# DeepRank/Deeprank-GNN

Measured on AMD Instinct MI355X. Metric: interface-graphs/sec (fwd+bwd) GINet batch=64 per GPU, higher is better.
Workload: dtype f32; 1 GPU; GINet train step (topology + body fwd + FC head/MSE + bwd + grad all-reduce + Adam) on SYN graphs: 200 nodes, ~1000 directed edges, 32 node feats, 50->16 clusters (BASELINE.json configs[1]); graphs_per_gpu=64, global_batch=64, parallelism=dp1, mode=native, step_layout=auto

## Files before the change

deeprank-gnn_amd/csrc/drgnn_capi.hip:

```cpp
#define DRGNN_KERNELS_MAIN
#include "drgnn_kernels.h"

#include <vector>
#include <algorithm>
#include <memory>
#include <string.h>
#include <stdlib.h>
#ifdef DRGNN_EMU
#define DRGNN_LDS_LIMIT (160 * 1024)
#else
#define DRGNN_LDS_LIMIT (160 * 1024)
#define HIP_TRY(expr)                                   \
    do {                                                \
        hipError_t e_ = (expr);                         \
        if (e_ != hipSuccess) return (int)e_;           \
    } while (0)
#endif



extern "C" {

int drgnn_abi_version(void) { return DRGNN_ABI_VERSION; }

// ... 1477 lines not shown
        if (int rc = head_width_check(d)) return rc;
    }
    if (int rc = net_check(d.net)) return rc;
    if (!d.g_conv1 || !d.g_conv2 || slabs_check(d.net, c.slabs.slabs_per_graph)) return DRGNN_E_ARG;
    if (c.cohort) return 0;
    if (c.options) { if (int rc = optim_check(c.optim)) return rc; }
    if (!c.slabs.conv_partials || !c.slabs.head_partials || !c.flat.grad) return DRGNN_E_ARG;
    if (d.compact && (!c.slabs.readout || !c.step2)) return DRGNN_E_ARG;
    if (c.apply_adam && (!c.flat.param || !c.flat.exp_avg || !c.flat.exp_avg_sq || (!d.compact && !c.step))) return DRGNN_E_ARG;
    return 0;
}
static void reduce_fill(ReduceArgs& r, const drgnn_net_desc* net, const float* partials, int64_t rows, const drgnn_conv_grads* g1,
                        const drgnn_conv_grads* g2) {
    r = ReduceArgs{};
    r.partials = partials; r.n_graphs = (int)rows; r.n_branch = net->n_branch;
    r.n_feat = net->n_feat; r.n_partial = (int)net_partial_floats(net->n_feat); r.kind = net->kind;
    for (int b = 0; b < DRGNN_MAX_BRANCH; ++b) { r.lay1[b] = net->conv1[b]; r.lay2[b] = net->conv2[b]; }
    for (int b = 0; b < net->n_branch; ++b) { r.g1[b] = g1[b]; r.g2[b] = g2[b]; }
}
static int update_sums_fill(UpdateArgs& u, const UpdateDst& d, const UpdateSlabs& s, int n_tail) {
    reduce_fill(u.r, d.net, s.conv_partials, slabs_split(d.net, s.slabs_per_graph) ? 2 * s.n_graphs : s.n_graphs, d.g_conv1, d.g_conv2);
    u.h.partials = s.head_partials; u.h.n_wg = (int)s.head_slabs;
    u.h.P = (int)(d.compact ? head_compact_floats(d.R, d.H, d.O) : head_partial_floats(d.R, d.H, d.O));
    u.readout = s.readout; u.hR = d.R; u.hH = d.H;
    u.blocks_per_branch = (u.r.n_partial + 63) / 64;
    u.conv_blocks = d.net->n_branch * u.blocks_per_branch;
    return (d.compact ? d.H * d.R : 0) + u.h.P - n_tail;
}

static int update_run(const UpdateCall& c) {
    if (int rc = update_check(c)) return rc;
    UpdateArgs u = {};
    const int head_items = update_sums_fill(u, c.dst, c.slabs, 1);
    const int n_blocks = u.conv_blocks + (head_items + 63) / 64;
    if (!c.cohort) { u.h.grad = c.flat.grad + c.flat.head_offset; u.ad.step = c.dst.compact ? c.step2 + 1 : c.step; }
    u.h.loss = c.loss; u.loss2 = (c.loss || c.cohort) ? c.loss2 : nullptr; u.step2 = c.dst.compact ? c.step2 : nullptr;
    u.ad.param = c.flat.param; u.ad.grad = c.flat.grad; u.ad.exp_avg = c.flat.exp_avg; u.ad.exp_avg_sq = c.flat.exp_avg_sq;
    u.ad.n = c.flat.n_param;
    const drgnn_optim* opt = c.apply_adam ? c.optim : nullptr;
    const bool opt_flat = opt && (opt->clip || optim_coupled(opt));
    if (c.optim) optim_adam_args(u.ad, c.optim);
    else adam_set_hyper(u.ad, c.lr, c.beta1, c.beta2, c.eps, 0.0);
    u.apply_adam = (c.apply_adam && !opt_flat) ? 1 : 0;
#ifdef DRGNN_EMU
    if (c.cohort) return DRGNN_E_CAPACITY;
    if (opt) u.apply_adam = 0;
    const ReduceArgs& r = u.r;
    for (int64_t i = 0; i < (int64_t)r.n_branch * r.n_partial; ++i) {
        const int br = (int)(i / r.n_partial), p = (int)(i % r.n_partial);
        if (!reduce_live(r, p)) continue;
        float* d = reduce_dst(r, br, p);
        if (d) update_store(u, d, reduce_sum(r, br, p, 0, 1));
    }
    for (int i = 0; i < head_items; ++i) update_head_store(u, i, update_head_sum(u, i, 0, 1));
    if (u.step2) u.step2[0] = u.step2[1];
    if (opt) return adam_opt_impl(u.ad, c.flat.grad, opt, 0, c.stream);
#else
    const dim3 grid((unsigned)n_blocks, c.cohort ? (unsigned)c.K : 1u), threads(DRGNN_UPDATE_THREADS);
    hipStream_t stream = (hipStream_t)c.stream;
    if (opt) {
        const bool words = opt->clip && !optim_coupled(opt);
        if (words && n_blocks > opt->norm_cap) return DRGNN_E_CAPACITY;
        hipLaunchKernelGGL(k_update_opt, grid, threads, 0, stream, u, *opt, words ? opt->norm_words : (double*)nullptr);
        HIP_TRY(hipGetLastError());
        return opt_flat ? adam_opt_impl(u.ad, c.flat.grad, opt, words ? n_blocks : 0, c.stream) : 0;
    }
    if (c.optims) {
        if (c.any_clip && n_blocks > drgnn_optim_norm_words(c.flat.n_param)) return DRGNN_E_CAPACITY;
// ... 44 lines not shown
    return 0;
}

extern "C" {

int drgnn_net_reduce_grads(const drgnn_net_desc* net, const float* partials, int64_t n_nodes, int64_t n_graphs,
                           drgnn_conv_grads* g_conv1, drgnn_conv_grads* g_conv2, float* grad_x, void* stream_) {
    if (int rc = net_check(net)) return rc;
    if (!partials || !g_conv1 || !g_conv2) return DRGNN_E_ARG;
    ReduceArgs r;
    reduce_fill(r, net, partials, n_graphs, g_conv1, g_conv2);
    r.grad_x = grad_x; r.n_nodes = n_nodes;
    int64_t items = (int64_t)net->n_branch * r.n_partial;
    if (grad_x && net->n_branch > 1 && n_nodes * net->n_feat > items) items = n_nodes * net->n_feat;
#ifdef DRGNN_EMU
    for (int64_t i = 0; i < (int64_t)net->n_branch * r.n_partial; ++i) {
        const int br = (int)(i / r.n_partial), p = (int)(i % r.n_partial);
        if (reduce_live(r, p)) reduce_write(r, br, p, reduce_sum(r, br, p, 0, 1));
    }
    for (int64_t i = 0; grad_x && i < n_nodes * net->n_feat; ++i) reduce_grad_x(r, i);
    (void)stream_; (void)items;
#else
    const int reduce_blocks = net->n_branch * ((r.n_partial + 63) / 64);
    hipLaunchKernelGGL(k_reduce, dim3((unsigned)reduce_blocks), dim3(256), 0, (hipStream_t)stream_, r, items);
    HIP_TRY(hipGetLastError());
#endif
    return 0;
}

int drgnn_train_update(const drgnn_net_desc* net, const float* conv_partials, int64_t n_graphs, drgnn_conv_grads* g_conv1,
                       drgnn_conv_grads* g_conv2, const float* head_partials, int64_t head_slabs, int32_t R, int32_t H, int32_t O,
                       int64_t head_offset, float* flat_param, float* flat_grad, float* exp_avg, float* exp_avg_sq, int64_t n_param,
                       const int32_t* step, float* loss, double lr, double beta1, double beta2, double eps, int32_t apply_adam,
                       void* stream_) {
    UpdateCall c = update_call({net, g_conv1, g_conv2, R, H, O, false}, {conv_partials, n_graphs, head_partials, head_slabs, nullptr, 0},
                               {flat_param, flat_grad, exp_avg, exp_avg_sq, n_param, head_offset}, loss, apply_adam, stream_);
    c.step = step; c.lr = lr; c.beta1 = beta1; c.beta2 = beta2; c.eps = eps;
    return update_run(c);
// ... 43 lines not shown
int drgnn_cohort_update(const drgnn_net_desc* net, const drgnn_cohort_member* members, int32_t K, const int32_t* counts,
                        drgnn_conv_grads* g_conv1, drgnn_conv_grads* g_conv2, int32_t R, int32_t H, int32_t O,
                        int64_t head_offset, int64_t n_param, float* losses, int32_t apply_adam, void* stream_) {
    return update_run(cohort_call({net, g_conv1, g_conv2, R, H, O, true}, {nullptr, nullptr, nullptr, nullptr, n_param, head_offset},
                                  members, K, counts, losses, apply_adam, stream_));
}

int drgnn_cohort_update_opt(const drgnn_net_desc* net, const drgnn_cohort_member* members, const drgnn_optim* optims, int32_t K,
                            const int32_t* counts, drgnn_conv_grads* g_conv1, drgnn_conv_grads* g_conv2, int32_t R, int32_t H,
                            int32_t O, int64_t head_offset, int64_t n_param, float* losses, int32_t apply_adam, int32_t any_clip,
                            void* stream_) {
    UpdateCall c = cohort_call({net, g_conv1, g_conv2, R, H, O, true}, {nullptr, nullptr, nullptr, nullptr, n_param, head_offset},
                               members, K, counts, losses, apply_adam, stream_);
    c.optims = optims; c.options = true; c.any_clip = any_clip;
    return update_run(c);
}

int drgnn_step_gradients(const drgnn_net_desc* net, const float* conv_partials, int64_t n_graphs, drgnn_conv_grads* g_conv1,
                         drgnn_conv_grads* g_conv2, const float* head_partials, const float* readout, int32_t R, int32_t H, int32_t O,
                         float* head_grad, const float* graph_weight, float* const* zero_ptr, const int64_t* zero_len, int32_t n_zero,
                         int32_t* step2, int32_t slabs_per_graph, void* stream_) {
    const UpdateDst dst = {net, g_conv1, g_conv2, R, H, O, true};
    int rc;
    if ((rc = net_check(net))) return rc;
    if (!conv_partials || !g_conv1 || !g_conv2 || !head_partials || !readout || !head_grad || n_graphs < 0) return DRGNN_E_ARG;
    if (n_zero < 0 || n_zero > DRGNN_ZERO_RANGES || (n_zero > 0 && (!zero_ptr || !zero_len))) return DRGNN_E_ARG;
    if ((rc = slabs_check(net, slabs_per_graph)) || (rc = head_width_check(dst))) return rc;
    GradArgs ga = {};
    UpdateArgs& u = ga.u;
    const int head_items = update_sums_fill(u, dst, {conv_partials, n_graphs, head_partials, n_graphs, readout, slabs_per_graph}, 2);
    const int head_blocks = (head_items + 63) / 64;
    u.h.grad = head_grad; u.step2 = step2;
    ga.graph_weight = graph_weight; ga.wshift = slabs_split(net, slabs_per_graph) ? 1 : 0; ga.n_zero = n_zero;
    for (int i = 0; i < n_zero; ++i) {
        if (!zero_ptr[i] || zero_len[i] < 0) return DRGNN_E_ARG;
        ga.zero_ptr[i] = zero_ptr[i]; ga.zero_len[i] = zero_len[i];
    }
#ifdef DRGNN_EMU
    const ReduceArgs& r = u.r;
    for (int64_t i = 0; i < (int64_t)net->n_branch * r.n_partial; ++i) {
        const int br = (int)(i / r.n_partial), p = (int)(i % r.n_partial);
        if (!reduce_live(r, p)) continue;
        float* d = reduce_dst(r, br, p);
        if (d) *d = graph_weight ? reduce_sum_w(r, br, p, 0, 1, graph_weight, ga.wshift) : reduce_sum(r, br, p, 0, 1);
    }
    for (int i = 0; i < head_items; ++i)
        head_grad[i] = graph_weight ? update_head_sum_w(u, i, 0, 1, graph_weight) : update_head_sum(u, i, 0, 1);
    for (int i = 0; i < n_zero; ++i) memset(ga.zero_ptr[i], 0, sizeof(float) * (size_t)ga.zero_len[i]);
    if (step2) step2[0] = step2[1];
    (void)stream_; (void)head_blocks;
#else
    hipLaunchKernelGGL(k_gradients, dim3((unsigned)(u.conv_blocks + head_blocks + 1)), dim3(256), 0, (hipStream_t)stream_, ga);
    HIP_TRY(hipGetLastError());
#endif
    return 0;
}

#ifdef DRGNN_EMU
#define DRGNN_GRID_ITEMS(kern, item_fn, n_items, stream, ...) \
    do { for (int64_t it_ = 0; it_ < (int64_t)(n_items); ++it_) item_fn(__VA_ARGS__, it_); (void)stream; } while (0)
#define DRGNN_GRID_BLOCKS(kern, block_fn, n_blocks, stream, ...) \
    do { for (int b_ = 0; b_ < (int)(n_blocks); ++b_) block_fn(__VA_ARGS__, b_); (void)stream; } while (0)
#else
#define DRGNN_GRID_ITEMS(kern, item_fn, n_items, stream, ...)                                              \
    do { if ((n_items) > 0) hipLaunchKernelGGL(kern, dim3((unsigned)(((n_items) + 255) / 256)), dim3(256), \
                                               0, (hipStream_t)(stream), __VA_ARGS__); } while (0)
#define DRGNN_GRID_BLOCKS(kern, block_fn, n_blocks, stream, ...)                                          \
// ... 1289 lines not shown
```

deeprank-gnn_amd/csrc/drgnn_head.h:

```cpp
#pragma once
#include "drgnn_net.h"

#define DRGNN_HEAD_TILE_SMALL 16
#define DRGNN_HEAD_TILE_LARGE 64
#define DRGNN_HEAD_TMP 4096

HD int head_tile(int64_t n_graphs) { return n_graphs <= 512 ? DRGNN_HEAD_TILE_SMALL : DRGNN_HEAD_TILE_LARGE; }

struct HeadArgs {
    const float* readout;
    const float* y_reg;
    const int64_t* y_cls;
    const float* class_w;
    const float* w1; const float* b1;
    const float* w2; const float* b2;
    const int32_t* step;
    float* pred;
    float* grad_readout;
    float* partials;
    int B, R, H, O, T;
    int HC;
    int task;
    int train;
    int sigmoid;
// ... 208 lines not shown
HD void adam_set_hyper(AdamArgs& a, double lr, double beta1, double beta2, double eps, double weight_decay) {
    a.lr = lr; a.beta1 = beta1; a.beta2 = beta2;
    a.beta2f = (float)beta2; a.omb1 = (float)(1.0 - beta1); a.omb2 = (float)(1.0 - beta2);
    a.eps = (float)eps; a.weight_decay = (float)weight_decay;
}

DEV double adam_ipow(double b, int t) {
    double r = 1.0;
    for (unsigned e = (unsigned)(t > 0 ? t : 0); e; e >>= 1) {
        if (e & 1u) r *= b;
        b *= b;
    }
    return r;
}
struct AdamPre { float p, m, v, step_size, sqrt_bc2; bool ok; float decay; };
template <bool OPT = false>
DEV void adam_bias_scalars(const AdamArgs& a, float& step_size, float& sqrt_bc2, const drgnn_optim* o = nullptr,
                           float* decay = nullptr) {
    const int t = a.step[0];
    const double bc1 = 1.0 - adam_ipow(a.beta1, t);
    const double bc2 = 1.0 - adam_ipow(a.beta2, t);
    if constexpr (OPT) {
        double lr = a.lr;
        if (o->lr_table && o->lr_n > 0) {
            const int e = (t < o->lr_n ? t : o->lr_n) - 1;
            lr = o->lr_table[e > 0 ? e : 0];
        }
        *decay = (float)(1.0 - lr * (o->decoupled ? o->weight_decay : 0.0));
        step_size = (float)(lr / bc1);
    } else {
        step_size = (float)(a.lr / bc1);
    }
    sqrt_bc2 = (float)sqrt(bc2);
}
DEV AdamPre adam_prefetch_state(const AdamArgs& a, int64_t i) {
    AdamPre r;
// ... 70 lines not shown
```

deeprank-gnn_amd/csrc/drgnn_kernels.h:

```cpp
#pragma once
#include "drgnn_head.h"
#include "drgnn_step.h"
#include "drgnn_step2.h"
#include "drgnn_step3.h"
#include "drgnn_layers.h"
#include "drgnn_mcl.h"
#include "drgnn_louvain.h"
#include "drgnn_iface.h"
#include "drgnn_score.h"
#include "drgnn_bsa.h"
#include "drgnn_hse.h"
#include "drgnn_depth.h"
#include "drgnn_posecluster.h"
#include "drgnn_fcc.h"
#include "drgnn_consensus.h"
#include "drgnn_rmsd.h"
#include "drgnn_pack.h"
#include "drgnn_metrics.h"
#include "drgnn_collate.h"
#include "drgnn_p2p.h"

struct PtrArgs {
    const int64_t* batch;
    const int64_t* edge_row;
// ... 202 lines not shown

struct ScanArgs { TopoView tv; int n_graphs; };
DEV void finalize_block(const ScanArgs& a, int* part) {
    const int B = a.n_graphs;
    const int src[3] = {DRGNN_TI_NC0, DRGNN_TI_NE1, DRGNN_TI_NC1};
    const int dst[3] = {DRGNN_TI_CPTR0, DRGNN_TI_E1PTR, DRGNN_TI_CPTR1};
    for (int w = 0; w < 3; ++w) {
        int32_t* out = a.tv.p[dst[w]];
        const int32_t* in = a.tv.p[src[w]];
        FOR_TID(i, B + 1) { out[i] = (i < B) ? in[i] : 0; }
        BARRIER();
        wg_exscan(out, B + 1, part);
    }
}

struct ReduceArgs {
    const float* partials;
    int n_graphs, n_branch, n_feat, n_partial;
    int kind;
    drgnn_conv_params lay1[DRGNN_MAX_BRANCH], lay2[DRGNN_MAX_BRANCH];
    drgnn_conv_grads g1[DRGNN_MAX_BRANCH], g2[DRGNN_MAX_BRANCH];
    float* grad_x; int64_t n_nodes;
};

DEV float* reduce_dst(const ReduceArgs& a, int br, int p) {
    const int F = a.n_feat;
    const int o_w1s = F * DRGNN_H1, o_b1 = 2 * F * DRGNN_H1, o_w2n = o_b1 + DRGNN_H1;
    const int o_w2s = o_w2n + DRGNN_H1 * DRGNN_H2, o_b2 = o_w2s + DRGNN_H1 * DRGNN_H2;
    if (p < o_w1s)
        return a.g1[br].w_nbr ? a.g1[br].w_nbr + (int64_t)(p / DRGNN_H1) * a.lay1[br].nbr_sk + (int64_t)(p % DRGNN_H1) * a.lay1[br].nbr_sh : nullptr;
    if (p < o_b1) {
        const int q = p - o_w1s;
        return a.g1[br].w_self ? a.g1[br].w_self + (int64_t)(q / DRGNN_H1) * a.lay1[br].self_sk + (int64_t)(q % DRGNN_H1) * a.lay1[br].self_sh : nullptr;
    }
    if (p < o_w2n) return a.g1[br].bias ? a.g1[br].bias + (p - o_b1) : nullptr;
    if (p < o_w2s) {
        const int q = p - o_w2n;
        return a.g2[br].w_nbr ? a.g2[br].w_nbr + (int64_t)(q / DRGNN_H2) * a.lay2[br].nbr_sk + (int64_t)(q % DRGNN_H2) * a.lay2[br].nbr_sh : nullptr;
    }
    if (p < o_b2) {
        const int q = p - o_w2s;
        return a.g2[br].w_self ? a.g2[br].w_self + (int64_t)(q / DRGNN_H2) * a.lay2[br].self_sk + (int64_t)(q % DRGNN_H2) * a.lay2[br].self_sh : nullptr;
    }
    return a.g2[br].bias ? a.g2[br].bias + (p - o_b2) : nullptr;
}
DEV void reduce_write(const ReduceArgs& a, int br, int p, float acc) {
    float* d = reduce_dst(a, br, p);
    if (d) *d = acc;
}

DEV bool reduce_live(const ReduceArgs& a, int p) {
    if (a.kind != DRGNN_GINET) return true;
    const int F = a.n_feat;
    const int o_w1s = F * DRGNN_H1, o_w2n = 2 * F * DRGNN_H1 + DRGNN_H1, o_w2s = o_w2n + DRGNN_H1 * DRGNN_H2;
    return p < o_w1s || (p >= o_w2n && p < o_w2s);
}

DEV float reduce_sum(const ReduceArgs& a, int br, int p, int first, int stride) {
    const float* src = a.partials + (int64_t)br * a.n_partial + p;
    const int64_t step = (int64_t)a.n_branch * a.n_partial;
    float acc = 0.0f;
    float v[16];
    int g = first;
    for (; g + 15 * stride < a.n_graphs; g += 16 * stride) {
#pragma unroll
        for (int k = 0; k < 16; ++k) v[k] = src[(int64_t)(g + k * stride) * step];
#pragma unroll
        for (int k = 0; k < 16; ++k) acc += v[k];
    }
    for (; g < a.n_graphs; g += stride) acc += src[(int64_t)g * step];
    return acc;
}

DEV float reduce_sum_w(const ReduceArgs& a, int br, int p, int first, int stride, const float* w, int wshift) {
    const float* src = a.partials + (int64_t)br * a.n_partial + p;
    const int64_t step = (int64_t)a.n_branch * a.n_partial;
    float acc = 0.0f;
    float v[16], c[16];
    int g = first;
    for (; g + 15 * stride < a.n_graphs; g += 16 * stride) {
#pragma unroll
        for (int k = 0; k < 16; ++k) { v[k] = src[(int64_t)(g + k * stride) * step]; c[k] = w[(g + k * stride) >> wshift]; }
#pragma unroll
        for (int k = 0; k < 16; ++k) acc = fmaf(c[k], v[k], acc);
    }
    for (; g < a.n_graphs; g += stride) acc = fmaf(w[g >> wshift], src[(int64_t)g * step], acc);
// ... 168 lines not shown
        if (TRAIN) {
            float* hp = A.hf.partials + (long)g * head_compact_floats(A.hf.R, A.hf.H, A.hf.O);
            FOR_TID(i, (int)head_compact_floats(A.hf.R, A.hf.H, A.hf.O)) { hp[i] = DRGNN_NAN; }
        }
        FOR_TID(o, A.hf.O) { A.hf.pred[(long)g * A.hf.O + o] = DRGNN_NAN; }
        return;
    }
    net_step3_graph_both<XF, GATHER, CLS, TRAIN, DUAL, SG>(A, d, g, gi, lds, L.capN, L.capE, L.capC, false, 0, 0, 0);
}
#endif

struct UpdateArgs {
    ReduceArgs r;
    HeadReduceArgs h;
    AdamArgs ad;
    int conv_blocks;
    int blocks_per_branch;
    int apply_adam;
    const float* readout;
    int hR, hH;
    int32_t* step2;
    float* loss2;
};

DEV void update_store(const UpdateArgs& u, float* dst, float g) {
    *dst = g;
    if (u.apply_adam) adam_item(u.ad, (int64_t)(dst - u.ad.grad));
}

DEV int update_head_items(const UpdateArgs& u) { return (u.readout ? u.hH * u.hR : 0) + u.h.P - 1; }
DEV float update_head_sum(const UpdateArgs& u, int item, int first, int stride) {
    float acc = 0.0f;
    if (u.readout) {
        const int HR = u.hH * u.hR;
        if (item < HR) {
            const int h = item / u.hR, r = item - h * u.hR;
            const float* dh = u.h.partials + h;
            const float* xr = u.readout + r;
            float va[16], vb[16];
            int w = first;
            for (; w + 15 * stride < u.h.n_wg; w += 16 * stride) {
#pragma unroll
                for (int k = 0; k < 16; ++k) { va[k] = dh[(long)(w + k * stride) * u.h.P]; vb[k] = xr[(long)(w + k * stride) * u.hR]; }
#pragma unroll
                for (int k = 0; k < 16; ++k) acc = fmaf(va[k], vb[k], acc);
            }
            for (; w < u.h.n_wg; w += stride) acc = fmaf(dh[(long)w * u.h.P], xr[(long)w * u.hR], acc);
            return acc;
        }
        item -= HR;
    }
// ... 2 lines not shown
    int w = first;
    for (; w + 15 * stride < u.h.n_wg; w += 16 * stride) {
#pragma unroll
        for (int k = 0; k < 16; ++k) v[k] = src[(long)(w + k * stride) * u.h.P];
#pragma unroll
        for (int k = 0; k < 16; ++k) acc += v[k];
    }
    for (; w < u.h.n_wg; w += stride) acc += src[(long)w * u.h.P];
    return acc;
}
DEV float update_head_sum_w(const UpdateArgs& u, int item, int first, int stride, const float* gw) {
    float acc = 0.0f;
    if (u.readout) {
        const int HR = u.hH * u.hR;
        if (item < HR) {
            const int h = item / u.hR, r = item - h * u.hR;
            const float* dh = u.h.partials + h;
            const float* xr = u.readout + r;
            float va[16], vb[16], vc[16];
            int w = first;
            for (; w + 15 * stride < u.h.n_wg; w += 16 * stride) {
#pragma unroll
                for (int k = 0; k < 16; ++k) {
                    va[k] = dh[(long)(w + k * stride) * u.h.P]; vb[k] = xr[(long)(w + k * stride) * u.hR]; vc[k] = gw[w + k * stride];
                }
#pragma unroll
                for (int k = 0; k < 16; ++k) acc = fmaf(vc[k] * va[k], vb[k], acc);
            }
            for (; w < u.h.n_wg; w += stride) acc = fmaf(gw[w] * dh[(long)w * u.h.P], xr[(long)w * u.hR], acc);
            return acc;
        }
// ... 44 lines not shown
    static_assert(N >= 1 && N <= 12, "lines per call");
    const char* base = (const char*)__builtin_amdgcn_kernarg_segment_ptr() + (off0 & ~63);
    int t;
#define DRGNN_KA_OFF(k) "i"(64 * ((k) < N ? (k) : N - 1))
    asm volatile("s_load_dword %0, %1, %2\n s_load_dword %0, %1, %3\n s_load_dword %0, %1, %4\n s_load_dword %0, %1, %5\n"
                 "s_load_dword %0, %1, %6\n s_load_dword %0, %1, %7\n s_load_dword %0, %1, %8\n s_load_dword %0, %1, %9\n"
                 "s_load_dword %0, %1, %10\n s_load_dword %0, %1, %11\n s_load_dword %0, %1, %12\n s_load_dword %0, %1, %13\n"
                 "s_waitcnt lgkmcnt(0)"
                 : "=&s"(t)
                 : "s"(base), DRGNN_KA_OFF(0), DRGNN_KA_OFF(1), DRGNN_KA_OFF(2), DRGNN_KA_OFF(3), DRGNN_KA_OFF(4), DRGNN_KA_OFF(5),
                   DRGNN_KA_OFF(6), DRGNN_KA_OFF(7), DRGNN_KA_OFF(8), DRGNN_KA_OFF(9), DRGNN_KA_OFF(10), DRGNN_KA_OFF(11)
                 : "memory");
#undef DRGNN_KA_OFF
}
#define DRGNN_KA_LINES(first_byte, end_byte) ((((end_byte) - 1) >> 6) - ((first_byte) >> 6) + 1)
template <bool LDS>
__global__ void __launch_bounds__(DRGNN_NTHREADS) k_topo(TopoLaunch L) {
    extern __shared__ __attribute__((aligned(16))) int smem_i[];
    PHASE_BEGIN();
    kernarg_touch_lines<DRGNN_KA_LINES(0, (int)sizeof(TopoLaunch))>(0);
    topo_block<LDS>(L, blockIdx.x, smem_i);
}
#ifdef DRGNN_KERNELS_MAIN
__global__ void __launch_bounds__(DRGNN_NTHREADS) k_tiles(TilesArgs a) { tiles_block(a, blockIdx.x); }
__global__ void __launch_bounds__(DRGNN_NTHREADS) k_finalize(ScanArgs a) {
    __shared__ int part[DRGNN_NTHREADS + 4];
    finalize_block(a, part);
}
__global__ void __launch_bounds__(256) k_reduce(ReduceArgs a, int64_t n_items) {
    __shared__ float quarter[4][64];
    const int lane = threadIdx.x & 63, q = threadIdx.x >> 6;
    const int bpb = (a.n_partial + 63) / 64;
    int br = 0, blk = (int)blockIdx.x;
    while (blk >= bpb && br + 1 < a.n_branch) { blk -= bpb; ++br; }
    const int p_raw = blk * 64 + lane;
    const bool live = p_raw < a.n_partial && reduce_live(a, p_raw);
    const int p = live ? p_raw : 0;
    quarter[q][lane] = live ? reduce_sum(a, br, p, q, 4) : 0.0f;
    __syncthreads();
    if (q == 0) {
        if (live) reduce_write(a, br, p, (quarter[0][lane] + quarter[1][lane]) + (quarter[2][lane] + quarter[3][lane]));
    } else {
        for (int64_t e = (int64_t)blockIdx.x * 192 + (threadIdx.x - 64); e < a.n_nodes * a.n_feat && a.grad_x; e += (int64_t)gridDim.x * 192)
            reduce_grad_x(a, e);
    }
}
#endif
template <int KIND, bool BWD, bool LDS>
__global__ void __launch_bounds__(DRGNN_NTHREADS) k_net(NetLaunch L) {
    extern __shared__ __attribute__((aligned(16))) float smem_f[];
    PHASE_BEGIN();
    net_block<KIND, BWD, LDS>(L, blockIdx.x, smem_f);
}
template <int KIND, bool BWD>
__global__ void __launch_bounds__(DRGNN_NTHREADS) k_net_co_topo(CoLaunch C) {
    extern __shared__ __attribute__((aligned(16))) float smem_c[];
// ... 302 lines not shown
    batch_offsets_block(a, blockIdx.x, smem_o + DRGNN_NTHREADS + 4, smem_o);
}
__global__ void __launch_bounds__(DRGNN_NTHREADS) k_collate(CollateArgs a) {
    __shared__ int sh[4];
    collate_block(a, blockIdx.x, sh);
}
__global__ void __launch_bounds__(DRGNN_NTHREADS) k_head(HeadArgs a) {
    extern __shared__ __attribute__((aligned(16))) float smem_h[];
    head_block(a, blockIdx.x, smem_h);
}
__global__ void __launch_bounds__(256) k_head_reduce(HeadReduceArgs a) {
    const int i = blockIdx.x * blockDim.x + threadIdx.x;
    if (i < a.P - 1) head_reduce_item(a, i);
}
#define DRGNN_UPDATE_THREADS 320
template <bool OPT>
DEV void update_block_t(const UpdateArgs& u, const ReduceArgs& dst, int blk_id, int64_t gshift, float (*quarter)[64], float* bias_scalars,
                        const drgnn_optim* o, double* words_out) {
    const int lane = threadIdx.x & 63, q = threadIdx.x >> 6;
    const bool conv = blk_id < u.conv_blocks;
    float* d = nullptr;
    bool upd = false, live = false;
    int64_t idx = -1;
    int item = 0, n_grad = 0;
    AdamPre pre;
    pre.ok = false; pre.p = pre.m = pre.v = 0.0f; pre.step_size = 0.0f; pre.sqrt_bc2 = 1.0f;
    if (q == 4) {
        if (lane == 0) {
            float step_size = 0.0f, sqrt_bc2 = 1.0f;
            float decay = 1.0f;
            if (u.apply_adam) adam_bias_scalars<OPT>(u.ad, step_size, sqrt_bc2, o, &decay);
            bias_scalars[0] = step_size; bias_scalars[1] = sqrt_bc2;
            if (OPT) bias_scalars[2] = decay;
        }
    } else if (conv) {
        const ReduceArgs& a = u.r;
        int br = 0, blk = blk_id;
        while (blk >= u.blocks_per_branch && br + 1 < a.n_branch) { blk -= u.blocks_per_branch; ++br; }
        const int p_raw = blk * 64 + lane;
        live = p_raw < a.n_partial && reduce_live(dst, p_raw);
        const int p = live ? p_raw : 0;
        d = (q == 0 && live) ? reduce_dst(dst, br, p) : nullptr;
        if (d) d += gshift;
        upd = d != nullptr && u.apply_adam;
        idx = upd ? (int64_t)(d - u.ad.grad) : -1;
        pre = adam_prefetch_state(u.ad, idx);
        quarter[q][lane] = live ? reduce_sum(a, br, p, q, 4) : 0.0f;
    } else {
        item = (blk_id - u.conv_blocks) * 64 + lane;
        live = item < update_head_items(u);
        n_grad = update_head_items(u) - 1;
        d = (q == 0 && live && item < n_grad) ? u.h.grad + item : nullptr;
        upd = d != nullptr && u.apply_adam;
        idx = upd ? (int64_t)(d - u.ad.grad) : -1;
        pre = adam_prefetch_state(u.ad, idx);
        quarter[q][lane] = live ? update_head_sum(u, item, q, 4) : 0.0f;
    }
    __syncthreads();
    if (q == 0) {
        pre.step_size = bias_scalars[0]; pre.sqrt_bc2 = bias_scalars[1];
        if (OPT) pre.decay = bias_scalars[2];
        const float g = (quarter[0][lane] + quarter[1][lane]) + (quarter[2][lane] + quarter[3][lane]);
        if (OPT && words_out) {
            double sq = d ? (double)g * (double)g : 0.0;
            for (int mask = 32; mask > 0; mask >>= 1) sq += __shfl_xor(sq, mask, 64);
            if (lane == 0) words_out[blk_id] = sq;
        }
        if (d) {
            *d = g;
            if (upd) adam_apply<OPT>(u.ad, idx, g, pre);
        } else if (!conv && live && item == n_grad && u.h.loss) {
            u.h.loss[0] = g;
            if (u.loss2) u.loss2[0] = g;
        }
    }
    if (u.step2 && blk_id == 0 && threadIdx.x == 0) u.step2[0] = u.step2[1];
}
DEV void update_block(const UpdateArgs& u, const ReduceArgs& dst, int blk_id, int64_t gshift, float (*quarter)[64], float* bias_scalars) {
    update_block_t<false>(u, dst, blk_id, gshift, quarter, bias_scalars, nullptr, nullptr);
}
__global__ void __launch_bounds__(DRGNN_UPDATE_THREADS) k_update(UpdateArgs u) {
    kernarg_touch_lines<DRGNN_KA_LINES(0, (int)sizeof(UpdateArgs))>(0);
    __shared__ float quarter[4][64];
    __shared__ float bias_scalars[2];
    update_block(u, u.r, (int)blockIdx.x, 0, quarter, bias_scalars);
}
__global__ void __launch_bounds__(DRGNN_UPDATE_THREADS) k_update_opt(UpdateArgs u, drgnn_optim o, double* words_out) {
    __shared__ float quarter[4][64];
    __shared__ float bias_scalars[3];
    update_block_t<true>(u, u.r, (int)blockIdx.x, 0, quarter, bias_scalars, &o, words_out);
}
__global__ void __launch_bounds__(DRGNN_UPDATE_THREADS) k_update_cohort(UpdateArgs u_by_value, const drgnn_cohort_member* members,
                                                                         const int32_t* counts, int64_t head_offset) {
    kernarg_touch_lines<DRGNN_KA_LINES(0, (int)sizeof(UpdateArgs))>(0);
    __shared__ float quarter[4][64];
    __shared__ float bias_scalars[2];
    const UpdateArgs& u0 = *reinterpret_cast<const UpdateArgs*>((const char*)__builtin_amdgcn_kernarg_segment_ptr());
    const int m = (int)blockIdx.y;
    const int B = __builtin_amdgcn_readfirstlane(counts[m]);
    if (B <= 0) return;
    const drgnn_cohort_member mm = wg_uniform_words(members[m]);
    UpdateArgs u = u0;
    u.r.partials = mm.partials; u.r.n_graphs = B;
    u.h.partials = mm.head_partials; u.h.n_wg = B;
    u.h.grad = mm.flat_grad + head_offset; u.h.loss = mm.loss;
    u.readout = mm.readout; u.step2 = mm.step2; u.loss2 = u0.loss2 ? u0.loss2 + m : nullptr;
    u.ad.param = mm.flat_param; u.ad.grad = mm.flat_grad; u.ad.exp_avg = mm.exp_avg; u.ad.exp_avg_sq = mm.exp_avg_sq;
    u.ad.step = mm.step2 + 1;
    adam_set_hyper(u.ad, mm.lr, mm.beta1, mm.beta2, mm.eps, 0.0);
// ... 63 lines not shown
                                                         const int32_t* counts, int64_t n_param, int n_words) {
    __shared__ AdamOptScalars sc;
    __shared__ double stage[256];
    const int m = (int)blockIdx.y;
    if (__builtin_amdgcn_readfirstlane(counts[m]) <= 0) return;
    const drgnn_optim& o = optims[m];
    if (!__builtin_amdgcn_readfirstlane(o.clip)) return;
    AdamArgs a;
    a.param = members[m].flat_param; a.grad = members[m].flat_grad; a.exp_avg = members[m].exp_avg;
    a.exp_avg_sq = members[m].exp_avg_sq; a.step = members[m].step2 + 1; a.n = n_param;
    adam_set_hyper(a, o.lr, o.beta1, o.beta2, o.eps, 0.0);
    adam_opt_block_scalars(a, o, n_words < o.norm_cap ? n_words : o.norm_cap, sc, stage);
    adam_opt_item(a, o, members[m].flat_grad, (int64_t)blockIdx.x * blockDim.x + threadIdx.x, sc);
}
__global__ void __launch_bounds__(256) k_gradients(GradArgs ga) {
    kernarg_touch_lines<DRGNN_KA_LINES(0, (int)sizeof(GradArgs))>(0);
    __shared__ float quarter[4][64];
    const UpdateArgs& u = ga.u;
    const int lane = threadIdx.x & 63, q = threadIdx.x >> 6;
    const int n_sum = u.conv_blocks + (update_head_items(u) - 1 + 63) / 64;
    if ((int)blockIdx.x >= n_sum) {
        for (int r = 0; r < ga.n_zero; ++r)
            for (int64_t i = threadIdx.x; i < ga.zero_len[r]; i += 256) ga.zero_ptr[r][i] = 0.0f;
        if (u.step2 && threadIdx.x == 0) u.step2[0] = u.step2[1];
        return;
    }
    const bool conv = (int)blockIdx.x < u.conv_blocks;
    const float* gw = ga.graph_weight;
    float* d = nullptr;
    bool live = false;
    if (conv) {
        const ReduceArgs& a = u.r;
        int br = 0, blk = (int)blockIdx.x;
        while (blk >= u.blocks_per_branch && br + 1 < a.n_branch) { blk -= u.blocks_per_branch; ++br; }
        const int p_raw = blk * 64 + lane;
        live = p_raw < a.n_partial && reduce_live(a, p_raw);
        const int p = live ? p_raw : 0;
        d = (q == 0 && live) ? reduce_dst(a, br, p) : nullptr;
        quarter[q][lane] = !live ? 0.0f : gw ? reduce_sum_w(a, br, p, q, 4, gw, ga.wshift) : reduce_sum(a, br, p, q, 4);
    } else {
        const int item = ((int)blockIdx.x - u.conv_blocks) * 64 + lane;
        live = item < update_head_items(u) - 1;
        d = (q == 0 && live) ? u.h.grad + item : nullptr;
        quarter[q][lane] = !live ? 0.0f : gw ? update_head_sum_w(u, item, q, 4, gw) : update_head_sum(u, item, q, 4);
    }
    __syncthreads();
    if (d) *d = (quarter[0][lane] + quarter[1][lane]) + (quarter[2][lane] + quarter[3][lane]);
}
__global__ void __launch_bounds__(DRGNN_P2P_THREADS) k_allreduce_oneshot(P2PArgs a) { p2p_block(a, blockIdx.x); }
__global__ void __launch_bounds__(256) k_adam(AdamArgs a) {
    adam_item(a, (int64_t)blockIdx.x * blockDim.x + threadIdx.x);
}
__global__ void __launch_bounds__(256) k_adam_opt(AdamArgs a, drgnn_optim o, float* grad, int n_words) {
    __shared__ AdamOptScalars sc;
    __shared__ double stage[256];
    adam_opt_block_scalars(a, o, n_words, sc, stage);
// ... 27 lines not shown
```

Baseline: 3.758 million graphs/s.

## Compact conv gradient reduction into precomputed live segments, skipping dead GINet slots

Host-side reduce_fill now builds a table of live gradient segments (base pointer, strides, slot offset, block start). Kernels map each block to a segment with a uniform compare scan instead of per-lane branchy offset decoding and liveness checks. For GINet this drops the blocks that covered w_self and bias slots, which were launched but did nothing. It also adds a dual-power Adam bias computation, shift-based head index math, a 16-line kernarg prefetch and scalar-register hints. The kernel argument struct grows with the segment table, and a segments query API is added.

```diff
diff --git a/deeprank-gnn_amd/csrc/drgnn_capi.hip b/deeprank-gnn_amd/csrc/drgnn_capi.hip
--- a/deeprank-gnn_amd/csrc/drgnn_capi.hip
+++ b/deeprank-gnn_amd/csrc/drgnn_capi.hip
@@ -1515,17 +1515,50 @@
                         const drgnn_conv_grads* g2) {
     r = ReduceArgs{};
     r.partials = partials; r.n_graphs = (int)rows; r.n_branch = net->n_branch;
-    r.n_feat = net->n_feat; r.n_partial = (int)net_partial_floats(net->n_feat); r.kind = net->kind;
-    for (int b = 0; b < DRGNN_MAX_BRANCH; ++b) { r.lay1[b] = net->conv1[b]; r.lay2[b] = net->conv2[b]; }
-    for (int b = 0; b < net->n_branch; ++b) { r.g1[b] = g1[b]; r.g2[b] = g2[b]; }
-}
+    r.n_feat = net->n_feat; r.n_partial = (int)net_partial_floats(net->n_feat);
+    const bool gin = net->kind == DRGNN_GINET;
+    const int F = net->n_feat;
+    for (int b = 0; b < net->n_branch; ++b) {
+        const drgnn_conv_params& l1 = net->conv1[b];
+        const drgnn_conv_params& l2 = net->conv2[b];
+        int slot = 0;
+        auto add = [&](float* base, int64_t sk, int64_t sh, int count, int lw, bool written) {
+            if (base && written && count > 0) {
+                GradSeg& g = r.seg[r.n_seg++];
+                g.base = base; g.sk = sk; g.sh = sh; g.slot0 = slot; g.count = count; g.blk0 = r.conv_blocks; g.br = b; g.lw = lw;
+                r.conv_blocks += (count + 63) / 64;
+            }
+            slot += count;
+        };
+        add(g1[b].w_nbr, l1.nbr_sk, l1.nbr_sh, F * DRGNN_H1, DRGNN_H1_LOG2, true);
+        add(g1[b].w_self, l1.self_sk, l1.self_sh, F * DRGNN_H1, DRGNN_H1_LOG2, !gin);
+        add(g1[b].bias, 0, 1, DRGNN_H1, DRGNN_H1_LOG2, !gin);
+        add(g2[b].w_nbr, l2.nbr_sk, l2.nbr_sh, DRGNN_H1 * DRGNN_H2, DRGNN_H2_LOG2, true);
+        add(g2[b].w_self, l2.self_sk, l2.self_sh, DRGNN_H1 * DRGNN_H2, DRGNN_H2_LOG2, !gin);
+        add(g2[b].bias, 0, 1, DRGNN_H2, DRGNN_H2_LOG2, !gin);
+    }
+    for (int s = r.n_seg; s < DRGNN_MAX_SEG; ++s) r.seg[s].blk0 = INT_MAX;
+}
+#ifdef DRGNN_EMU
+template <class Fn>
+static void reduce_walk(const ReduceArgs& r, Fn fn) {
+    for (int s = 0; s < r.n_seg; ++s) {
+        const int blk1 = s + 1 < r.n_seg ? r.seg[s + 1].blk0 : r.conv_blocks;
+        for (int blk = r.seg[s].blk0; blk < blk1; ++blk)
+            for (int lane = 0; lane < 64; ++lane) {
+                const SegLane L = seg_lane(r, blk, lane);
+                if (L.live) fn(L);
+            }
+    }
+}
+#endif
 static int update_sums_fill(UpdateArgs& u, const UpdateDst& d, const UpdateSlabs& s, int n_tail) {
     reduce_fill(u.r, d.net, s.conv_partials, slabs_split(d.net, s.slabs_per_graph) ? 2 * s.n_graphs : s.n_graphs, d.g_conv1, d.g_conv2);
     u.h.partials = s.head_partials; u.h.n_wg = (int)s.head_slabs;
     u.h.P = (int)(d.compact ? head_compact_floats(d.R, d.H, d.O) : head_partial_floats(d.R, d.H, d.O));
     u.readout = s.readout; u.hR = d.R; u.hH = d.H;
-    u.blocks_per_branch = (u.r.n_partial + 63) / 64;
-    u.conv_blocks = d.net->n_branch * u.blocks_per_branch;
+    u.hR_log2 = -1;
+    for (int k = 0; k < 31; ++k) if (d.R == (1 << k)) u.hR_log2 = k;
     return (d.compact ? d.H * d.R : 0) + u.h.P - n_tail;
 }
 
@@ -1533,7 +1566,7 @@
     if (int rc = update_check(c)) return rc;
     UpdateArgs u = {};
     const int head_items = update_sums_fill(u, c.dst, c.slabs, 1);
-    const int n_blocks = u.conv_blocks + (head_items + 63) / 64;
+    const int n_blocks = u.r.conv_blocks + (head_items + 63) / 64;
     if (!c.cohort) { u.h.grad = c.flat.grad + c.flat.head_offset; u.ad.step = c.dst.compact ? c.step2 + 1 : c.step; }
     u.h.loss = c.loss; u.loss2 = (c.loss || c.cohort) ? c.loss2 : nullptr; u.step2 = c.dst.compact ? c.step2 : nullptr;
     u.ad.param = c.flat.param; u.ad.grad = c.flat.grad; u.ad.exp_avg = c.flat.exp_avg; u.ad.exp_avg_sq = c.flat.exp_avg_sq;
@@ -1547,12 +1580,7 @@
     if (c.cohort) return DRGNN_E_CAPACITY;
     if (opt) u.apply_adam = 0;
     const ReduceArgs& r = u.r;
-    for (int64_t i = 0; i < (int64_t)r.n_branch * r.n_partial; ++i) {
-        const int br = (int)(i / r.n_partial), p = (int)(i % r.n_partial);
-        if (!reduce_live(r, p)) continue;
-        float* d = reduce_dst(r, br, p);
-        if (d) update_store(u, d, reduce_sum(r, br, p, 0, 1));
-    }
+    reduce_walk(r, [&](const SegLane& L) { update_store(u, L.d, reduce_sum(r, L.br, L.p, 0, 1)); });
     for (int i = 0; i < head_items; ++i) update_head_store(u, i, update_head_sum(u, i, 0, 1));
     if (u.step2) u.step2[0] = u.step2[1];
     if (opt) return adam_opt_impl(u.ad, c.flat.grad, opt, 0, c.stream);
@@ -1627,14 +1655,11 @@
     int64_t items = (int64_t)net->n_branch * r.n_partial;
     if (grad_x && net->n_branch > 1 && n_nodes * net->n_feat > items) items = n_nodes * net->n_feat;
 #ifdef DRGNN_EMU
-    for (int64_t i = 0; i < (int64_t)net->n_branch * r.n_partial; ++i) {
-        const int br = (int)(i / r.n_partial), p = (int)(i % r.n_partial);
-        if (reduce_live(r, p)) reduce_write(r, br, p, reduce_sum(r, br, p, 0, 1));
-    }
+    reduce_walk(r, [&](const SegLane& L) { *L.d = reduce_sum(r, L.br, L.p, 0, 1); });
     for (int64_t i = 0; grad_x && i < n_nodes * net->n_feat; ++i) reduce_grad_x(r, i);
     (void)stream_; (void)items;
 #else
-    const int reduce_blocks = net->n_branch * ((r.n_partial + 63) / 64);
+    const int reduce_blocks = r.conv_blocks > 0 ? r.conv_blocks : 1;
     hipLaunchKernelGGL(k_reduce, dim3((unsigned)reduce_blocks), dim3(256), 0, (hipStream_t)stream_, r, items);
     HIP_TRY(hipGetLastError());
 #endif
@@ -1708,6 +1733,21 @@
                                members, K, counts, losses, apply_adam, stream_);
     c.optims = optims; c.options = true; c.any_clip = any_clip;
     return update_run(c);
+}
+
+int drgnn_update_segments(const drgnn_net_desc* net, const drgnn_conv_grads* g_conv1, const drgnn_conv_grads* g_conv2, int64_t* out,
+                          int32_t cap) {
+    if (int rc = net_check(net)) return rc;
+    if (!g_conv1 || !g_conv2 || !out || cap < 1 + 8 * DRGNN_MAX_SEG) return DRGNN_E_ARG;
+    ReduceArgs r;
+    reduce_fill(r, net, nullptr, 0, g_conv1, g_conv2);
+    out[0] = r.conv_blocks;
+    for (int s = 0; s < r.n_seg; ++s) {
+        const GradSeg& g = r.seg[s];
+        const int64_t w[8] = {(int64_t)(intptr_t)g.base, g.sk, g.sh, g.slot0, g.count, g.blk0, g.br, g.lw};
+        for (int k = 0; k < 8; ++k) out[1 + 8 * s + k] = w[k];
+    }
+    return r.n_seg;
 }
 
 int drgnn_step_gradients(const drgnn_net_desc* net, const float* conv_partials, int64_t n_graphs, drgnn_conv_grads* g_conv1,
@@ -1732,19 +1772,16 @@
     }
 #ifdef DRGNN_EMU
     const ReduceArgs& r = u.r;
-    for (int64_t i = 0; i < (int64_t)net->n_branch * r.n_partial; ++i) {
-        const int br = (int)(i / r.n_partial), p = (int)(i % r.n_partial);
-        if (!reduce_live(r, p)) continue;
-        float* d = reduce_dst(r, br, p);
-        if (d) *d = graph_weight ? reduce_sum_w(r, br, p, 0, 1, graph_weight, ga.wshift) : reduce_sum(r, br, p, 0, 1);
-    }
+    reduce_walk(r, [&](const SegLane& L) {
+        *L.d = graph_weight ? reduce_sum_w(r, L.br, L.p, 0, 1, graph_weight, ga.wshift) : reduce_sum(r, L.br, L.p, 0, 1);
+    });
     for (int i = 0; i < head_items; ++i)
         head_grad[i] = graph_weight ? update_head_sum_w(u, i, 0, 1, graph_weight) : update_head_sum(u, i, 0, 1);
     for (int i = 0; i < n_zero; ++i) memset(ga.zero_ptr[i], 0, sizeof(float) * (size_t)ga.zero_len[i]);
     if (step2) step2[0] = step2[1];
     (void)stream_; (void)head_blocks;
 #else
-    hipLaunchKernelGGL(k_gradients, dim3((unsigned)(u.conv_blocks + head_blocks + 1)), dim3(256), 0, (hipStream_t)stream_, ga);
+    hipLaunchKernelGGL(k_gradients, dim3((unsigned)(u.r.conv_blocks + head_blocks + 1)), dim3(256), 0, (hipStream_t)stream_, ga);
     HIP_TRY(hipGetLastError());
 #endif
     return 0;
diff --git a/deeprank-gnn_amd/csrc/drgnn_head.h b/deeprank-gnn_amd/csrc/drgnn_head.h
--- a/deeprank-gnn_amd/csrc/drgnn_head.h
+++ b/deeprank-gnn_amd/csrc/drgnn_head.h
@@ -246,12 +246,21 @@
     return r;
 }
 struct AdamPre { float p, m, v, step_size, sqrt_bc2; bool ok; float decay; };
+DEV void adam_ipow2(double b1, double b2, int t, double& r1, double& r2) {
+    r1 = 1.0; r2 = 1.0;
+    for (unsigned e = (unsigned)(t > 0 ? t : 0); e; e >>= 1) {
+        if (e & 1u) { r1 *= b1; r2 *= b2; }
+        b1 *= b1; b2 *= b2;
+    }
+}
 template <bool OPT = false>
 DEV void adam_bias_scalars(const AdamArgs& a, float& step_size, float& sqrt_bc2, const drgnn_optim* o = nullptr,
                            float* decay = nullptr) {
     const int t = a.step[0];
-    const double bc1 = 1.0 - adam_ipow(a.beta1, t);
-    const double bc2 = 1.0 - adam_ipow(a.beta2, t);
+    double p1, p2;
+    adam_ipow2(a.beta1, a.beta2, t, p1, p2);
+    const double bc1 = 1.0 - p1;
+    const double bc2 = 1.0 - p2;
     if constexpr (OPT) {
         double lr = a.lr;
         if (o->lr_table && o->lr_n > 0) {
diff --git a/deeprank-gnn_amd/csrc/drgnn_kernels.h b/deeprank-gnn_amd/csrc/drgnn_kernels.h
--- a/deeprank-gnn_amd/csrc/drgnn_kernels.h
+++ b/deeprank-gnn_amd/csrc/drgnn_kernels.h
@@ -240,49 +240,52 @@
     }
 }
 
+#define DRGNN_H1_LOG2 4
+#define DRGNN_H2_LOG2 5
+static_assert((1 << DRGNN_H1_LOG2) == DRGNN_H1 && (1 << DRGNN_H2_LOG2) == DRGNN_H2, "row widths of the conv gradients");
+#define DRGNN_MAX_SEG (6 * DRGNN_MAX_BRANCH)
+struct GradSeg {
+    float* base; int64_t sk, sh;
+    int slot0, count;
+    int blk0;
+    int br, lw, reserved;
+};
 struct ReduceArgs {
     const float* partials;
     int n_graphs, n_branch, n_feat, n_partial;
-    int kind;
-    drgnn_conv_params lay1[DRGNN_MAX_BRANCH], lay2[DRGNN_MAX_BRANCH];
-    drgnn_conv_grads g1[DRGNN_MAX_BRANCH], g2[DRGNN_MAX_BRANCH];
+    int n_seg, conv_blocks;
+    GradSeg seg[DRGNN_MAX_SEG];
     float* grad_x; int64_t n_nodes;
 };
 
-DEV float* reduce_dst(const ReduceArgs& a, int br, int p) {
-    const int F = a.n_feat;
-    const int o_w1s = F * DRGNN_H1, o_b1 = 2 * F * DRGNN_H1, o_w2n = o_b1 + DRGNN_H1;
-    const int o_w2s = o_w2n + DRGNN_H1 * DRGNN_H2, o_b2 = o_w2s + DRGNN_H1 * DRGNN_H2;
-    if (p < o_w1s)
-        return a.g1[br].w_nbr ? a.g1[br].w_nbr + (int64_t)(p / DRGNN_H1) * a.lay1[br].nbr_sk + (int64_t)(p % DRGNN_H1) * a.lay1[br].nbr_sh : nullptr;
-    if (p < o_b1) {
-        const int q = p - o_w1s;
-        return a.g1[br].w_self ? a.g1[br].w_self + (int64_t)(q / DRGNN_H1) * a.lay1[br].self_sk + (int64_t)(q % DRGNN_H1) * a.lay1[br].self_sh : nullptr;
-    }
-    if (p < o_w2n) return a.g1[br].bias ? a.g1[br].bias + (p - o_b1) : nullptr;
-    if (p < o_w2s) {
-        const int q = p - o_w2n;
-        return a.g2[br].w_nbr ? a.g2[br].w_nbr + (int64_t)(q / DRGNN_H2) * a.lay2[br].nbr_sk + (int64_t)(q % DRGNN_H2) * a.lay2[br].nbr_sh : nullptr;
-    }
-    if (p < o_b2) {
-        const int q = p - o_w2s;
-        return a.g2[br].w_self ? a.g2[br].w_self + (int64_t)(q / DRGNN_H2) * a.lay2[br].self_sk + (int64_t)(q % DRGNN_H2) * a.lay2[br].self_sh : nullptr;
-    }
-    return a.g2[br].bias ? a.g2[br].bias + (p - o_b2) : nullptr;
-}
-DEV void reduce_write(const ReduceArgs& a, int br, int p, float acc) {
-    float* d = reduce_dst(a, br, p);
-    if (d) *d = acc;
-}
-
-DEV bool reduce_live(const ReduceArgs& a, int p) {
-    if (a.kind != DRGNN_GINET) return true;
-    const int F = a.n_feat;
-    const int o_w1s = F * DRGNN_H1, o_w2n = 2 * F * DRGNN_H1 + DRGNN_H1, o_w2s = o_w2n + DRGNN_H1 * DRGNN_H2;
-    return p < o_w1s || (p >= o_w2n && p < o_w2s);
-}
-
-DEV float reduce_sum(const ReduceArgs& a, int br, int p, int first, int stride) {
+struct SegIds { int blk0[DRGNN_MAX_SEG]; };
+DEV SegIds seg_ids(const ReduceArgs& a) {
+    SegIds ids;
+#pragma unroll
+    for (int k = 0; k < DRGNN_MAX_SEG; ++k) ids.blk0[k] = a.seg[k].blk0;
+    return ids;
+}
+DEV int seg_of_block(const SegIds& ids, int blk) {
+    int s = 0;
+#pragma unroll
+    for (int k = 1; k < DRGNN_MAX_SEG; ++k) s += (blk >= ids.blk0[k]) ? 1 : 0;
+    return WG_UNIFORM(s);
+}
+struct SegLane { bool live; int br, p; float* d; };
+DEV SegLane seg_lane(const ReduceArgs& a, int s, int blk, int lane) {
+    const GradSeg g = a.seg[s];
+    const int i_raw = (blk - g.blk0) * 64 + lane;
+    SegLane L;
+    L.live = i_raw < g.count;
+    const int i = L.live ? i_raw : 0;
+    L.br = g.br; L.p = g.slot0 + i;
+    L.d = g.base + (int64_t)(i >> g.lw) * g.sk + (int64_t)(i & ((1 << g.lw) - 1)) * g.sh;
+    return L;
+}
+DEV SegLane seg_lane(const ReduceArgs& a, int blk, int lane) { return seg_lane(a, seg_of_block(seg_ids(a), blk), blk, lane); }
+
+struct ReduceSrc { const float* partials; int n_graphs, n_branch, n_partial; };
+DEV float reduce_sum(const ReduceSrc& a, int br, int p, int first, int stride) {
     const float* src = a.partials + (int64_t)br * a.n_partial + p;
     const int64_t step = (int64_t)a.n_branch * a.n_partial;
     float acc = 0.0f;
@@ -296,6 +299,11 @@
     }
     for (; g < a.n_graphs; g += stride) acc += src[(int64_t)g * step];
     return acc;
+}
+
+DEV float reduce_sum(const ReduceArgs& a, int br, int p, int first, int stride) {
+    const ReduceSrc s = {a.partials, a.n_graphs, a.n_branch, a.n_partial};
+    return reduce_sum(s, br, p, first, stride);
 }
 
 DEV float reduce_sum_w(const ReduceArgs& a, int br, int p, int first, int stride, const float* w, int wshift) {
@@ -494,11 +502,10 @@
     ReduceArgs r;
     HeadReduceArgs h;
     AdamArgs ad;
-    int conv_blocks;
-    int blocks_per_branch;
     int apply_adam;
     const float* readout;
     int hR, hH;
+    int hR_log2;
     int32_t* step2;
     float* loss2;
 };
@@ -509,12 +516,17 @@
 }
 
 DEV int update_head_items(const UpdateArgs& u) { return (u.readout ? u.hH * u.hR : 0) + u.h.P - 1; }
+DEV void update_head_hr(const UpdateArgs& u, int item, int& h, int& r) {
+    if (u.hR_log2 >= 0) { h = item >> u.hR_log2; r = item & (u.hR - 1); }
+    else { h = item / u.hR; r = item - h * u.hR; }
+}
 DEV float update_head_sum(const UpdateArgs& u, int item, int first, int stride) {
     float acc = 0.0f;
     if (u.readout) {
         const int HR = u.hH * u.hR;
         if (item < HR) {
-            const int h = item / u.hR, r = item - h * u.hR;
+            int h, r;
+            update_head_hr(u, item, h, r);
             const float* dh = u.h.partials + h;
             const float* xr = u.readout + r;
             float va[16], vb[16];
@@ -547,7 +559,8 @@
     if (u.readout) {
         const int HR = u.hH * u.hR;
         if (item < HR) {
-            const int h = item / u.hR, r = item - h * u.hR;
+            int h, r;
+            update_head_hr(u, item, h, r);
             const float* dh = u.h.partials + h;
             const float* xr = u.readout + r;
             float va[16], vb[16], vc[16];
@@ -622,6 +635,30 @@
 #undef DRGNN_KA_OFF
 }
 #define DRGNN_KA_LINES(first_byte, end_byte) ((((end_byte) - 1) >> 6) - ((first_byte) >> 6) + 1)
+template <int N>
+DEV void kernarg_touch_lines16(int off0) {
+    static_assert(N >= 13 && N <= 16, "lines per call");
+    const char* base = (const char*)__builtin_amdgcn_kernarg_segment_ptr() + (off0 & ~63);
+    int t;
+#define DRGNN_KA_OFF(k) "i"(64 * ((k) < N ? (k) : N - 1))
+    asm volatile("s_load_dword %0, %1, %2\n s_load_dword %0, %1, %3\n s_load_dword %0, %1, %4\n s_load_dword %0, %1, %5\n"
+                 "s_load_dword %0, %1, %6\n s_load_dword %0, %1, %7\n s_load_dword %0, %1, %8\n s_load_dword %0, %1, %9\n"
+                 "s_load_dword %0, %1, %10\n s_load_dword %0, %1, %11\n s_load_dword %0, %1, %12\n s_load_dword %0, %1, %13\n"
+                 "s_load_dword %0, %1, %14\n s_load_dword %0, %1, %15\n s_load_dword %0, %1, %16\n s_load_dword %0, %1, %17\n"
+                 "s_waitcnt lgkmcnt(0)"
+                 : "=&s"(t)
+                 : "s"(base), DRGNN_KA_OFF(0), DRGNN_KA_OFF(1), DRGNN_KA_OFF(2), DRGNN_KA_OFF(3), DRGNN_KA_OFF(4), DRGNN_KA_OFF(5),
+                   DRGNN_KA_OFF(6), DRGNN_KA_OFF(7), DRGNN_KA_OFF(8), DRGNN_KA_OFF(9), DRGNN_KA_OFF(10), DRGNN_KA_OFF(11),
+                   DRGNN_KA_OFF(12), DRGNN_KA_OFF(13), DRGNN_KA_OFF(14), DRGNN_KA_OFF(15)
+                 : "memory");
+#undef DRGNN_KA_OFF
+}
+template <int BYTES>
+DEV void kernarg_touch_args() {
+    constexpr int N = DRGNN_KA_LINES(0, BYTES);
+    if constexpr (N <= 12) kernarg_touch_lines<N>(0);
+    else kernarg_touch_lines16<(N < 16 ? N : 16)>(0);
+}
 template <bool LDS>
 __global__ void __launch_bounds__(DRGNN_NTHREADS) k_topo(TopoLaunch L) {
     extern __shared__ __attribute__((aligned(16))) int smem_i[];
@@ -638,16 +675,13 @@
 __global__ void __launch_bounds__(256) k_reduce(ReduceArgs a, int64_t n_items) {
     __shared__ float quarter[4][64];
     const int lane = threadIdx.x & 63, q = threadIdx.x >> 6;
-    const int bpb = (a.n_partial + 63) / 64;
-    int br = 0, blk = (int)blockIdx.x;
-    while (blk >= bpb && br + 1 < a.n_branch) { blk -= bpb; ++br; }
-    const int p_raw = blk * 64 + lane;
-    const bool live = p_raw < a.n_partial && reduce_live(a, p_raw);
-    const int p = live ? p_raw : 0;
-    quarter[q][lane] = live ? reduce_sum(a, br, p, q, 4) : 0.0f;
+    SegLane L;
+    L.live = false; L.br = L.p = 0; L.d = nullptr;
+    if ((int)blockIdx.x < a.conv_blocks) L = seg_lane(a, (int)blockIdx.x, lane);
+    quarter[q][lane] = L.live ? reduce_sum(a, L.br, L.p, q, 4) : 0.0f;
     __syncthreads();
     if (q == 0) {
-        if (live) reduce_write(a, br, p, (quarter[0][lane] + quarter[1][lane]) + (quarter[2][lane] + quarter[3][lane]));
+        if (L.live) *L.d = (quarter[0][lane] + quarter[1][lane]) + (quarter[2][lane] + quarter[3][lane]);
     } else {
         for (int64_t e = (int64_t)blockIdx.x * 192 + (threadIdx.x - 64); e < a.n_nodes * a.n_feat && a.grad_x; e += (int64_t)gridDim.x * 192)
             reduce_grad_x(a, e);
@@ -980,11 +1014,28 @@
     if (i < a.P - 1) head_reduce_item(a, i);
 }
 #define DRGNN_UPDATE_THREADS 320
+struct AdamBufs { float* param; const float* grad; float* exp_avg; float* exp_avg_sq; int64_t n; int apply; };
+DEV AdamPre adam_prefetch_state(const AdamBufs& b, int64_t i) {
+    AdamPre r;
+    r.ok = i >= 0 && i < b.n;
+    r.p = r.m = r.v = 0.0f; r.step_size = 0.0f; r.sqrt_bc2 = 1.0f; r.decay = 1.0f;
+    if (!r.ok) return r;
+    r.p = b.param[i];
+    r.m = b.exp_avg[i];
+    r.v = b.exp_avg_sq[i];
+    return r;
+}
+#ifdef DRGNN_EMU
+#define DRGNN_SCALARS_NOW(...) ((void)0)
+#else
+#define DRGNN_SCALARS_NOW(...) asm volatile("" : : __VA_ARGS__)
+#endif
+#define DRGNN_ADAM_BUFS_S(ab) "s"(ab.param), "s"(ab.grad), "s"(ab.exp_avg), "s"(ab.exp_avg_sq), "s"(ab.n), "s"(ab.apply)
 template <bool OPT>
 DEV void update_block_t(const UpdateArgs& u, const ReduceArgs& dst, int blk_id, int64_t gshift, float (*quarter)[64], float* bias_scalars,
                         const drgnn_optim* o, double* words_out) {
     const int lane = threadIdx.x & 63, q = threadIdx.x >> 6;
-    const bool conv = blk_id < u.conv_blocks;
+    const bool conv = blk_id < dst.conv_blocks;
     float* d = nullptr;
     bool upd = false, live = false;
     int64_t idx = -1;
@@ -992,6 +1043,7 @@
     AdamPre pre;
     pre.ok = false; pre.p = pre.m = pre.v = 0.0f; pre.step_size = 0.0f; pre.sqrt_bc2 = 1.0f;
     if (q == 4) {
+        DRGNN_SCALARS_NOW("s"(u.apply_adam), "s"(u.ad.step), "s"(u.ad.lr), "s"(u.ad.beta1), "s"(u.ad.beta2));
         if (lane == 0) {
             float step_size = 0.0f, sqrt_bc2 = 1.0f;
             float decay = 1.0f;
@@ -1000,26 +1052,31 @@
             if (OPT) bias_scalars[2] = decay;
         }
     } else if (conv) {
-        const ReduceArgs& a = u.r;
-        int br = 0, blk = blk_id;
-        while (blk >= u.blocks_per_branch && br + 1 < a.n_branch) { blk -= u.blocks_per_branch; ++br; }
-        const int p_raw = blk * 64 + lane;
-        live = p_raw < a.n_partial && reduce_live(dst, p_raw);
-        const int p = live ? p_raw : 0;
-        d = (q == 0 && live) ? reduce_dst(dst, br, p) : nullptr;
-        if (d) d += gshift;
-        upd = d != nullptr && u.apply_adam;
-        idx = upd ? (int64_t)(d - u.ad.grad) : -1;
-        pre = adam_prefetch_state(u.ad, idx);
-        quarter[q][lane] = live ? reduce_sum(a, br, p, q, 4) : 0.0f;
+        const ReduceSrc src = {u.r.partials, u.r.n_graphs, u.r.n_branch, u.r.n_partial};
+        const AdamBufs ab = {u.ad.param, u.ad.grad, u.ad.exp_avg, u.ad.exp_avg_sq, u.ad.n, u.apply_adam};
+        const SegIds ids = seg_ids(dst);
+        DRGNN_SCALARS_NOW("s"(src.partials), "s"(src.n_graphs), "s"(src.n_branch), "s"(src.n_partial), DRGNN_ADAM_BUFS_S(ab),
+                          "s"(ids.blk0[1]), "s"(ids.blk0[2]), "s"(ids.blk0[3]), "s"(ids.blk0[4]), "s"(ids.blk0[5]), "s"(ids.blk0[6]),
+                          "s"(ids.blk0[7]), "s"(ids.blk0[8]), "s"(ids.blk0[9]), "s"(ids.blk0[10]), "s"(ids.blk0[11]));
+        static_assert(DRGNN_MAX_SEG == 12, "the first-block ids above");
+        const SegLane L = seg_lane(dst, seg_of_block(ids, blk_id), blk_id, lane);
+        live = L.live;
+        d = (q == 0 && live) ? L.d + gshift : nullptr;
+        upd = d != nullptr && ab.apply;
+        idx = upd ? (int64_t)(d - ab.grad) : -1;
+        pre = adam_prefetch_state(ab, idx);
+        quarter[q][lane] = live ? reduce_sum(src, L.br, L.p, q, 4) : 0.0f;
     } else {
-        item = (blk_id - u.conv_blocks) * 64 + lane;
+        const AdamBufs ab = {u.ad.param, u.ad.grad, u.ad.exp_avg, u.ad.exp_avg_sq, u.ad.n, u.apply_adam};
+        DRGNN_SCALARS_NOW(DRGNN_ADAM_BUFS_S(ab), "s"(u.h.partials), "s"(u.h.n_wg), "s"(u.h.P), "s"(u.h.grad), "s"(u.readout),
+                          "s"(u.hR), "s"(u.hH), "s"(u.hR_log2));
+        item = (blk_id - dst.conv_blocks) * 64 + lane;
         live = item < update_head_items(u);
         n_grad = update_head_items(u) - 1;
         d = (q == 0 && live && item < n_grad) ? u.h.grad + item : nullptr;
-        upd = d != nullptr && u.apply_adam;
-        idx = upd ? (int64_t)(d - u.ad.grad) : -1;
-        pre = adam_prefetch_state(u.ad, idx);
+        upd = d != nullptr && ab.apply;
+        idx = upd ? (int64_t)(d - ab.grad) : -1;
+        pre = adam_prefetch_state(ab, idx);
         quarter[q][lane] = live ? update_head_sum(u, item, q, 4) : 0.0f;
     }
     __syncthreads();
@@ -1046,7 +1103,7 @@
     update_block_t<false>(u, dst, blk_id, gshift, quarter, bias_scalars, nullptr, nullptr);
 }
 __global__ void __launch_bounds__(DRGNN_UPDATE_THREADS) k_update(UpdateArgs u) {
-    kernarg_touch_lines<DRGNN_KA_LINES(0, (int)sizeof(UpdateArgs))>(0);
+    kernarg_touch_args<(int)sizeof(UpdateArgs)>();
     __shared__ float quarter[4][64];
     __shared__ float bias_scalars[2];
     update_block(u, u.r, (int)blockIdx.x, 0, quarter, bias_scalars);
@@ -1058,7 +1115,7 @@
 }
 __global__ void __launch_bounds__(DRGNN_UPDATE_THREADS) k_update_cohort(UpdateArgs u_by_value, const drgnn_cohort_member* members,
                                                                          const int32_t* counts, int64_t head_offset) {
-    kernarg_touch_lines<DRGNN_KA_LINES(0, (int)sizeof(UpdateArgs))>(0);
+    kernarg_touch_args<(int)sizeof(UpdateArgs)>();
     __shared__ float quarter[4][64];
     __shared__ float bias_scalars[2];
     const UpdateArgs& u0 = *reinterpret_cast<const UpdateArgs*>((const char*)__builtin_amdgcn_kernarg_segment_ptr());
@@ -1152,32 +1209,29 @@
     adam_opt_item(a, o, members[m].flat_grad, (int64_t)blockIdx.x * blockDim.x + threadIdx.x, sc);
 }
 __global__ void __launch_bounds__(256) k_gradients(GradArgs ga) {
-    kernarg_touch_lines<DRGNN_KA_LINES(0, (int)sizeof(GradArgs))>(0);
+    kernarg_touch_args<(int)sizeof(GradArgs)>();
     __shared__ float quarter[4][64];
     const UpdateArgs& u = ga.u;
     const int lane = threadIdx.x & 63, q = threadIdx.x >> 6;
-    const int n_sum = u.conv_blocks + (update_head_items(u) - 1 + 63) / 64;
+    const int n_sum = u.r.conv_blocks + (update_head_items(u) - 1 + 63) / 64;
     if ((int)blockIdx.x >= n_sum) {
         for (int r = 0; r < ga.n_zero; ++r)
             for (int64_t i = threadIdx.x; i < ga.zero_len[r]; i += 256) ga.zero_ptr[r][i] = 0.0f;
         if (u.step2 && threadIdx.x == 0) u.step2[0] = u.step2[1];
         return;
     }
-    const bool conv = (int)blockIdx.x < u.conv_blocks;
+    const bool conv = (int)blockIdx.x < u.r.conv_blocks;
     const float* gw = ga.graph_weight;
     float* d = nullptr;
     bool live = false;
     if (conv) {
         const ReduceArgs& a = u.r;
-        int br = 0, blk = (int)blockIdx.x;
-        while (blk >= u.blocks_per_branch && br + 1 < a.n_branch) { blk -= u.blocks_per_branch; ++br; }
-        const int p_raw = blk * 64 + lane;
-        live = p_raw < a.n_partial && reduce_live(a, p_raw);
-        const int p = live ? p_raw : 0;
-        d = (q == 0 && live) ? reduce_dst(a, br, p) : nullptr;
-        quarter[q][lane] = !live ? 0.0f : gw ? reduce_sum_w(a, br, p, q, 4, gw, ga.wshift) : reduce_sum(a, br, p, q, 4);
+        const SegLane L = seg_lane(a, (int)blockIdx.x, lane);
+        live = L.live;
+        d = (q == 0 && live) ? L.d : nullptr;
+        quarter[q][lane] = !live ? 0.0f : gw ? reduce_sum_w(a, L.br, L.p, q, 4, gw, ga.wshift) : reduce_sum(a, L.br, L.p, q, 4);
     } else {
-        const int item = ((int)blockIdx.x - u.conv_blocks) * 64 + lane;
+        const int item = ((int)blockIdx.x - u.r.conv_blocks) * 64 + lane;
         live = item < update_head_items(u) - 1;
         d = (q == 0 && live) ? u.h.grad + item : nullptr;
         quarter[q][lane] = !live ? 0.0f : gw ? update_head_sum_w(u, item, q, 4, gw) : update_head_sum(u, item, q, 4);
```

Result: no change. 3.775 million graphs/s, median of 6 (+0.4%).
